# brown-palm/goal-force

Measured on AMD Instinct MI355X. Metric: frames_per_sec (81-frame video / (50-step denoise loop + VAE decode), Wan2.2-I2V-A14B 832x480x81f), higher is better.
Workload: dtype bf16

## Files before the change

goal_force_amd/csrc/gf_abi.hip:

```cpp
#include "gf_common.h"
#include <cstdarg>
#include <cstdio>
#include <cstdlib>
#include <cstring>

static thread_local char g_err[512] = "";

void gf_set_error(const char* fmt, ...) {
    va_list ap;
    va_start(ap, fmt);
    vsnprintf(g_err, sizeof(g_err), fmt, ap);
    va_end(ap);
}

extern "C" GF_API const char* gf_version(void) { return "goalforce-hip 0.1.0 gfx950"; }
extern "C" GF_API const char* gf_last_error(void) { return g_err; }
extern "C" GF_API int gf_abi_version(void) { return GF_ABI_VERSION; }

static GfOptions g_options;

const GfOptions& gf_options() { return g_options; }

namespace {
struct OptionSlot {
    const char* name;
    std::atomic<int> GfOptions::*field;
    int lo, hi, dflt;
};
const OptionSlot kSlots[] = {
    {"prefer_8wave", &GfOptions::prefer_8wave, 0, 1, 0}, {"a4_stagger", &GfOptions::a4_stagger, 0, 1 << 20, 2},
    {"a4_group_m", &GfOptions::a4_group_m, 0, 64, 0},    {"conv_nb", &GfOptions::conv_nb, 0, 2, 0},
    {"conv_gather", &GfOptions::conv_gather, 0, 1, 0},   {"vae_rms3", &GfOptions::vae_rms3, 0, 1, 1},
    {"conv_direct", &GfOptions::conv_direct, 0, 1, 1},
};
}

extern "C" GF_API int gf_set_option(const char* name, int value) {
    GF_CHECK_ARG(name, "gf_set_option: null name");
    for (const OptionSlot& s : kSlots)
        if (strcmp(name, s.name) == 0) {
            (g_options.*(s.field)).store(value < s.lo ? s.lo : (value > s.hi ? s.hi : value), std::memory_order_relaxed);
            return GF_OK;
        }
    gf_set_error("gf_set_option: unknown option '%s'", name);
    return GF_ERR_INVALID_ARG;
}

extern "C" GF_API int gf_get_option(const char* name, int* value) {
    GF_CHECK_ARG(name && value, "gf_get_option: null argument");
    for (const OptionSlot& s : kSlots)
        if (strcmp(name, s.name) == 0) {
            *value = (g_options.*(s.field)).load(std::memory_order_relaxed);
            return GF_OK;
        }
    gf_set_error("gf_get_option: unknown option '%s'", name);
    return GF_ERR_INVALID_ARG;
}

extern "C" GF_API void gf_reset_options(void) {
    for (const OptionSlot& s : kSlots) (g_options.*(s.field)).store(s.dflt, std::memory_order_relaxed);
}
```

goal_force_amd/csrc/gf_common.h:

```cpp
#pragma once
#include <hip/hip_runtime.h>
#include <stdint.h>
#include "goalforce.h"

typedef unsigned short u16;
typedef __attribute__((ext_vector_type(8))) __bf16 bf16x8;
typedef __attribute__((ext_vector_type(4))) __bf16 bf16x4;
typedef __attribute__((ext_vector_type(8))) unsigned short u16x8;
typedef __attribute__((ext_vector_type(4))) unsigned short u16x4;
typedef __attribute__((ext_vector_type(4))) short s16x4;
typedef __attribute__((ext_vector_type(4))) float f32x4;
typedef __attribute__((ext_vector_type(16))) float f32x16;
typedef __attribute__((ext_vector_type(4))) unsigned int u32x4;
typedef __attribute__((ext_vector_type(2))) unsigned int u32x2;

#define GF_LDS __attribute__((address_space(3)))
#define GF_GLOBAL __attribute__((address_space(1)))

__device__ __forceinline__ float bf2f(u16 u) { return __uint_as_float(((unsigned)u) << 16); }
__device__ __forceinline__ u16 f2bf(float f) { return __builtin_bit_cast(u16, (__bf16)f); }
__device__ __forceinline__ float rbf(float f) { return bf2f(f2bf(f)); }
__device__ __forceinline__ unsigned pack2bf(float lo, float hi) {
    typedef __attribute__((ext_vector_type(2))) float f2_t;
    typedef __attribute__((ext_vector_type(2))) __bf16 b2_t;
    return __builtin_bit_cast(unsigned, __builtin_convertvector(f2_t{lo, hi}, b2_t));
}

__device__ __forceinline__ float gelu_tanh_f(float x) {
    const float a = -2.0f * 0.7978845608028654f * 1.4426950408889634f, b = a * 0.044715f;
    const float t = __builtin_amdgcn_exp2f(x * __builtin_fmaf(b, x * x, a));
    return x * __builtin_amdgcn_rcpf(1.0f + t);
}
typedef __attribute__((ext_vector_type(2))) float gf_f32x2;
__device__ __forceinline__ void gelu_tanh_f4(gf_f32x2& x01, gf_f32x2& x23) {
    const float a = -2.0f * 0.7978845608028654f * 1.4426950408889634f, b = a * 0.044715f;
    const gf_f32x2 av = {a, a}, bv = {b, b}, one = {1.0f, 1.0f};
    const gf_f32x2 g01 = x01 * __builtin_elementwise_fma(bv, x01 * x01, av), g23 = x23 * __builtin_elementwise_fma(bv, x23 * x23, av);
    const float t0 = __builtin_amdgcn_exp2f(g01[0]), t1 = __builtin_amdgcn_exp2f(g01[1]);
    const float t2 = __builtin_amdgcn_exp2f(g23[0]), t3 = __builtin_amdgcn_exp2f(g23[1]);
    const gf_f32x2 d01 = one + gf_f32x2{t0, t1}, d23 = one + gf_f32x2{t2, t3};
    const float r0 = __builtin_amdgcn_rcpf(d01[0]), r1 = __builtin_amdgcn_rcpf(d01[1]);
    const float r2 = __builtin_amdgcn_rcpf(d23[0]), r3 = __builtin_amdgcn_rcpf(d23[1]);
    x01 = x01 * gf_f32x2{r0, r1};
    x23 = x23 * gf_f32x2{r2, r3};
}
__device__ __forceinline__ float silu_f(float x) { return x / (1.0f + __expf(-x)); }

__device__ __forceinline__ float wave_sum(float v) {
#pragma unroll
    for (int o = 32; o > 0; o >>= 1) v += __shfl_xor(v, o);
    return v;
}

template <int THREADS>
__device__ __forceinline__ float block_sum(float v, float* red) {
    v = wave_sum(v);
    const int w = threadIdx.x >> 6;
    __syncthreads();
    if ((threadIdx.x & 63) == 0) red[w] = v;
    __syncthreads();
    float t = 0.f;
#pragma unroll
    for (int i = 0; i < THREADS / 64; ++i) t += red[i];
    return t;
}

void gf_set_error(const char* fmt, ...);
#define GF_CHECK_ARG(cond, ...)                 \
    do {                                        \
        if (!(cond)) {                          \
            gf_set_error(__VA_ARGS__);          \
            return GF_ERR_INVALID_ARG;          \
        }                                       \
    } while (0)
#define GF_CHECK_LAUNCH(name)                                                        \
    do {                                                                             \
        hipError_t e_ = hipGetLastError();                                           \
        if (e_ != hipSuccess) {                                                      \
            gf_set_error("%s: launch failed: %s", name, hipGetErrorString(e_));      \
            return GF_ERR_LAUNCH;                                                    \
        }                                                                            \
    } while (0)
static inline bool gf_aligned16(const void* p) { return (((uintptr_t)p) & 15u) == 0; }

#include <atomic>
struct GfOptions {
    std::atomic<int> prefer_8wave{0};
    std::atomic<int> a4_stagger{2};
    std::atomic<int> a4_group_m{0};
    std::atomic<int> conv_nb{0};
    std::atomic<int> conv_gather{0};
    std::atomic<int> vae_rms3{1};
    std::atomic<int> conv_direct{1};
};
int gf_conv3d_direct_c96(const void* src_walk, const void* Wm, int64_t ldw, const void* bias, void* out, int64_t T_out, int64_t H,
                         int64_t W, int64_t N, int epilogue, const void* resid, const void* zero_page, void* stream);
int gf_conv2d_up_direct_c192(const void* src0, const void* Wm, int64_t ldw, const void* bias, void* out, int64_t T_out, int64_t Hs,
                             int64_t Ws, const void* zero_page, void* stream);
const GfOptions& gf_options();

#include <atomic>
#include <mutex>
struct GfDeviceOnce {
    std::atomic<uint64_t> done{0};
    std::mutex mu;
};
template <class F>
static inline hipError_t gf_once_per_device(GfDeviceOnce& st, F&& f) {
    int dev = 0;
    hipError_t e = hipGetDevice(&dev);
    if (e != hipSuccess) return e;
    if (dev < 0 || dev >= 64) return hipErrorInvalidDevice;
    const uint64_t bit = 1ull << dev;
    if (st.done.load(std::memory_order_acquire) & bit) return hipSuccess;
    std::lock_guard<std::mutex> lock(st.mu);
    if (st.done.load(std::memory_order_relaxed) & bit) return hipSuccess;
    e = f();
    if (e == hipSuccess) st.done.fetch_or(bit, std::memory_order_release);
    return e;
}
```

goal_force_amd/csrc/gf_gemm.hip:

```cpp
#include "gf_common.h"
#include <cstdlib>
#include <type_traits>


namespace {

constexpr int BM = 256, BN = 256, BK = 64;
constexpr int GEMM_THREADS = 512;
constexpr int TILE_BYTES = BM * BK * 2;
constexpr int STAGE_BYTES = 2 * TILE_BYTES;
constexpr int GEMM_LDS = 2 * STAGE_BYTES;
constexpr int GROUP_M = 8;

struct ConvGeom {
    const u16* src;
    const u16* cache;
    const u16* zero;
    int H, W, C, Ho, Wo, kt, ks, mode, t_stride, t_off, taps;
    int hist_front;
    int c64;
    long frame;
    float inv_c, inv_ks2;
};

// ... 547 lines not shown
#pragma unroll
        for (int j = 0; j < 2; ++j) {
            if (b && j >= J1) continue;
            const int ncol = (NB == 3 && b) ? 128 + wc * 16 + fq * 4 : b * 128 + wc * 32 + j * 16 + fq * 4;
            float bv[4] = {0.f, 0.f, 0.f, 0.f};
            if (p.bias && n0 + ncol < p.N) {
                const u16x4 b4 = *reinterpret_cast<const u16x4*>(p.bias + n0 + ncol);
#pragma unroll
                for (int r = 0; r < 4; ++r) bv[r] = bf2f(b4[r]);
            }
#pragma unroll
            for (int a = 0; a < 2; ++a)
#pragma unroll
                for (int i = 0; i < 4; ++i) {
                    const int row = a * 128 + wr * 64 + i * 16 + frow;
                    float rs = 1.0f;
                    if constexpr (FP8) rs = p.row_scale[min(m0 + row, p.M - 1)];
                    float y[4];
#pragma unroll
                    for (int r = 0; r < 4; ++r) {
                        y[r] = gf_epi_act<EPI>(acc[a][b][i][j][r] * rs + bv[r]);
                    }
                    u32x2 pk;
                    pk[0] = pack2bf(y[0], y[1]);
                    pk[1] = pack2bf(y[2], y[3]);
                    const int slot = (ncol >> 2) ^ ((row & 15) << 1);
                    *(GF_LDS u32x2*)(lds + row * 512 + slot * 8) = pk;
                }
        }
    __syncthreads();
    {
        const int cc = lane & 31;
        const int n = n0 + cc * 8;
        const bool n_ok = n < p.N && cc * 8 < BNT;
        u16x8 g8;
        if (EPI == GF_EPI_BIAS_GATE_RESID && n_ok) g8 = *reinterpret_cast<const u16x8*>(p.gate + n);
#pragma unroll
        for (int it = 0; it < 16; ++it) {
            const int row = wave * 32 + it * 2 + (lane >> 5);
            const int m = m0 + row;
            const u16x8 yv = *(GF_LDS u16x8*)(lds + row * 512 + ((cc ^ (row & 15)) << 4));
            if (m < p.M && n_ok) {
                u16x8 o = yv;
                if (EPI == GF_EPI_BIAS_GATE_RESID || EPI == GF_EPI_BIAS_RESID || EPI == GF_EPI_BIAS_MUL) {
                    const u16x8 r8 = rpre[HAS_R ? it : 0];
#pragma unroll
                    for (int e = 0; e < 8; ++e) {
                        float t = bf2f(yv[e]);
                        if (EPI == GF_EPI_BIAS_GATE_RESID) t = rbf(bf2f(g8[e]) * t);
                        o[e] = (EPI == GF_EPI_BIAS_MUL) ? f2bf(t * bf2f(r8[e]))
                                                        : f2bf(bf2f(r8[e]) + t);
                    }
                }
                *reinterpret_cast<u16x8*>(pC + (long)m * p.ldc + n) = o;
            }
        }
    }
}

#include "gf_gemm_a4_loop.inc"
#include "gf_gemm_a4f8_loop.inc"
constexpr int A4_THREADS = 256;

template <int I>
__device__ __forceinline__ float a4_acc() {
    float x;
    asm volatile("v_accvgpr_read_b32 %0, a[%1]" : "=v"(x) : "n"(I));
    return x;
}
template <int I, int N, class F>
__device__ __forceinline__ void a4_static_for(F&& f) {
    if constexpr (I < N) {
        f(std::integral_constant<int, I>{});
        a4_static_for<I + 1, N>(f);
    }
}

template <int EPI, bool FP8 = false>
__global__ __launch_bounds__(A4_THREADS, 1) void gemm_a4_kernel(const GemmArgs p) {
    constexpr unsigned ESZ = FP8 ? 1u : 2u;
    extern __shared__ __attribute__((aligned(16))) char smem[];
    GF_LDS char* lds = (GF_LDS char*)smem;
    const int tid = threadIdx.x;
    const int lane = tid & 63;
    const int wave = __builtin_amdgcn_readfirstlane(tid >> 6);
    const int wm = wave >> 1, wn = wave & 1;

    const int nwg = p.tiles_m * p.tiles_n;
    int v;
    {
        const int pid = blockIdx.x;
        const int xcd = pid & 7, local = pid >> 3;
        const int q = nwg >> 3, r = nwg & 7;
        v = (xcd < r ? xcd * (q + 1) : r * (q + 1) + (xcd - r) * q) + local;
    }
    const int gm = p.group_m;
    const int per_group = gm * p.tiles_n;
    const int group = v / per_group;
    const int first_m = group * gm;
    const int gsz = min(p.tiles_m - first_m, gm);
    const int in_group = v - group * per_group;
    const int m0 = (first_m + in_group % gsz) * BM, n0 = (in_group / gsz) * BN;

    const int srow = lane >> 3;
    unsigned voffA = (unsigned)srow * (unsigned)p.lda * ESZ + (unsigned)(((lane & 7) ^ srow) << 4);
    unsigned voffB = (unsigned)srow * (unsigned)p.ldw * ESZ + (unsigned)(((lane & 7) ^ srow) << 4);
    unsigned pfA = (unsigned)lane * (unsigned)p.lda * ESZ, pfB = (unsigned)lane * (unsigned)p.ldw * ESZ;
    const unsigned long baseA = (unsigned long)((const char*)p.A + (long)m0 * p.lda * ESZ);
    const unsigned long baseB = (unsigned long)((const char*)p.W + (long)n0 * p.ldw * ESZ);
    const unsigned aLo = (unsigned)baseA, aHi = (unsigned)(baseA >> 32) & 0xffffu;
    const unsigned bLo = (unsigned)baseB, bHi = (unsigned)(baseB >> 32) & 0xffffu;
    const unsigned nrA = (unsigned)(((long)(min(p.M - m0, BM) - 1) * p.lda + p.K) * ESZ);
    const int wvalid = min(p.wrows - n0, BN);
    const unsigned nrB = wvalid > 0 ? (unsigned)(((long)(wvalid - 1) * p.ldw + p.K) * ESZ) : 0u;
    const unsigned stA = 32u * (unsigned)p.lda * ESZ, stB = 32u * (unsigned)p.ldw * ESZ;
    const unsigned soA = (unsigned)wave * 8u * (unsigned)p.lda * ESZ, soB = (unsigned)wave * 8u * (unsigned)p.ldw * ESZ;
    const unsigned ldsW = (unsigned)(unsigned long)lds + (unsigned)wave * 1024u;
    const unsigned nk = (unsigned)(p.K * (int)ESZ / 128);
    const unsigned k0 = p.stagger ? (unsigned)((p.stagger * (p.stagger_rows ? m0 / BM : n0 / BN)) % (int)nk) : 0u;
    const unsigned kb = (unsigned)p.K * ESZ;

    const int frow = lane & 15, fq = lane >> 4, sw = frow & 7;
    const unsigned lbase = (unsigned)(unsigned long)lds;
    unsigned rdA0 = lbase + (unsigned)((wm * 128 + frow) * 128 + (((0 + fq) ^ sw) << 4));
    unsigned rdA1 = lbase + (unsigned)((wm * 128 + frow) * 128 + (((4 + fq) ^ sw) << 4));
    unsigned rdB0 = lbase + (unsigned)(TILE_BYTES + (wn * 128 + frow) * 128 + (((0 + fq) ^ sw) << 4));
    unsigned rdB1 = lbase + (unsigned)(TILE_BYTES + (wn * 128 + frow) * 128 + (((4 + fq) ^ sw) << 4));

    u16x4 bpre[8];
    u16x8 gpre = {0, 0, 0, 0, 0, 0, 0, 0};
    {
        const int fq_ = lane >> 4;
#pragma unroll
        for (int j = 0; j < 8; ++j) {
            const int n = n0 + wn * 128 + j * 16 + fq_ * 4;
            bpre[j] = (EPI != GF_EPI_VT32 && p.bias && n < p.N) ? *reinterpret_cast<const u16x4*>(p.bias + n) : u16x4{0, 0, 0, 0};
        }
        const int ng = n0 + wn * 128 + (lane & 15) * 8;
        if (EPI == GF_EPI_BIAS_GATE_RESID && ng < p.N) gpre = *reinterpret_cast<const u16x8*>(p.gate + ng);
        if (EPI == GF_EPI_VT32 && p.bias) {
#pragma unroll
            for (int i = 0; i < 8; ++i) {
                const int mrow = m0 + wm * 128 + i * 16 + (lane & 15);
                if (mrow < p.M) bpre[i][0] = p.bias[mrow];
            }
        }
    }
    float rsc[FP8 ? 8 : 1];
    if constexpr (FP8 && EPI != GF_EPI_VT32) {
#pragma unroll
        for (int i = 0; i < 8; ++i) rsc[i] = p.row_scale[min(m0 + wm * 128 + i * 16 + (lane & 15), p.M - 1)];
    }
    if constexpr (FP8) {
        GF_A4F8_LOOP_ASM(voffA, voffB, rdA0, rdA1, rdB0, rdB1, aLo, aHi, nrA, bLo, bHi, nrB, soA, stA, soB, stB, ldsW, nk, k0, kb);
    } else
    {
        GF_A4_LOOP_ASM(voffA, voffB, pfA, pfB, rdA0, rdA1, rdB0, rdB1, aLo, aHi, nrA, bLo, bHi, nrB, soA, stA, soB, stB, ldsW, nk, k0, kb);
    }

    GF_LDS char* ep = lds + wave * 32768;
    constexpr bool HAS_R = EPI == GF_EPI_BIAS_GATE_RESID || EPI == GF_EPI_BIAS_RESID || EPI == GF_EPI_BIAS_MUL;
    u16x8 rres[HAS_R ? 32 : 1];
    if constexpr (HAS_R) {
        const int nr = n0 + wn * 128 + (lane & 15) * 8;
#pragma unroll
        for (int it = 0; it < 32; ++it) {
            const int mr = m0 + wm * 128 + it * 4 + (lane >> 4);
            if (mr < p.M && nr < p.N) {
                rres[it] = __builtin_nontemporal_load(reinterpret_cast<const u16x8*>(p.R + (long)mr * p.ldr + nr));
            } else {
                rres[it] = u16x8{0, 0, 0, 0, 0, 0, 0, 0};
            }
        }
    }
    f32x4 csc[(FP8 && EPI == GF_EPI_VT32) ? 8 : 1];
    if constexpr (FP8 && EPI == GF_EPI_VT32) {
#pragma unroll
        for (int j = 0; j < 8; ++j) {
            const int n = n0 + wn * 128 + j * 16 + fq * 4;
#pragma unroll
            for (int r = 0; r < 4; ++r) csc[j][r] = (n + r < p.wrows) ? p.row_scale[n + r] : 0.f;
        }
    }
    a4_static_for<0, 8>([&](auto j_c) {
        constexpr int j = decltype(j_c)::value;
        const int n = n0 + wn * 128 + j * 16 + fq * 4;
        const float bv[4] = {bf2f(bpre[j][0]), bf2f(bpre[j][1]), bf2f(bpre[j][2]), bf2f(bpre[j][3])};
        a4_static_for<0, 8>([&](auto i_c) {
            constexpr int i = decltype(i_c)::value;
            constexpr int A0 = (i * 8 + j) * 4;
            float y[4] = {a4_acc<A0>(), a4_acc<A0 + 1>(), a4_acc<A0 + 2>(), a4_acc<A0 + 3>()};
            if constexpr (FP8 && EPI != GF_EPI_VT32) {
#pragma unroll
                for (int r = 0; r < 4; ++r) y[r] = y[r] * rsc[i] + bv[r];
            }
            if constexpr (EPI == GF_EPI_VT32) {
                const float bm = bf2f(bpre[i][0]);
                if constexpr (FP8) {
#pragma unroll
                    for (int r = 0; r < 4; ++r) y[r] = (n + r < p.wrows) ? y[r] * csc[j][r] + bm : 0.f;
                } else {
#pragma unroll
                    for (int r = 0; r < 4; ++r) y[r] = (n + r < p.wrows) ? y[r] + bm : 0.f;
                }
            } else if constexpr (EPI == GF_EPI_BIAS_GELU_TANH) {
                const unsigned l01 = FP8 ? pack2bf(y[0], y[1]) : pack2bf(y[0] + bv[0], y[1] + bv[1]);
                const unsigned l23 = FP8 ? pack2bf(y[2], y[3]) : pack2bf(y[2] + bv[2], y[3] + bv[3]);
                gf_f32x2 g01 = {__uint_as_float(l01 << 16), __uint_as_float(l01 & 0xffff0000u)};
                gf_f32x2 g23 = {__uint_as_float(l23 << 16), __uint_as_float(l23 & 0xffff0000u)};
                gelu_tanh_f4(g01, g23);
                y[0] = g01[0];
                y[1] = g01[1];
                y[2] = g23[0];
                y[3] = g23[1];
            } else {
#pragma unroll
                for (int r = 0; r < 4; ++r) {
                    y[r] = gf_epi_act<EPI>(FP8 ? y[r] : y[r] + bv[r]);
                }
            }
            u32x2 pk;
            pk[0] = pack2bf(y[0], y[1]);
            pk[1] = pack2bf(y[2], y[3]);
            const int row = i * 16 + frow;
            const int slot = (j * 4 + fq) ^ ((row & 15) << 1);
            *(GF_LDS u32x2*)(ep + row * 256 + slot * 8) = pk;
        });
    });
    asm volatile("s_waitcnt lgkmcnt(0)" ::: "memory");
    {
        const int cc = lane & 15;
        const int n = n0 + wn * 128 + cc * 8;
        const bool n_ok = n < p.N;
        const u16x8 g8 = gpre;
#pragma unroll
        for (int it = 0; it < 32; ++it) {
            const int row = it * 4 + (lane >> 4);
            const int m = m0 + wm * 128 + row;
            u16x8 yv;
            if constexpr (EPI == GF_EPI_VT32) {
                const int G = cc >> 2, g = cc & 3, sw = (row & 15) << 1;
                const u16x4 lo = *(GF_LDS u16x4*)(ep + row * 256 + (((8 * G + g) ^ sw) << 3));
                const u16x4 hi = *(GF_LDS u16x4*)(ep + row * 256 + (((8 * G + 4 + g) ^ sw) << 3));
                yv = u16x8{lo[0], lo[1], lo[2], lo[3], hi[0], hi[1], hi[2], hi[3]};
            } else {
                yv = *(GF_LDS u16x8*)(ep + row * 256 + ((cc ^ (row & 15)) << 4));
            }
            if (m < p.M && n_ok) {
                u16x8 o = yv;
                if constexpr (HAS_R) {
                    const u16x8 r8 = rres[it];
#pragma unroll
                    for (int e = 0; e < 8; ++e) {
                        float t = bf2f(yv[e]);
                        if (EPI == GF_EPI_BIAS_GATE_RESID) t = rbf(bf2f(g8[e]) * t);
                        o[e] = (EPI == GF_EPI_BIAS_MUL) ? f2bf(t * bf2f(r8[e]))
                                                        : f2bf(bf2f(r8[e]) + t);
                    }
                }
                __builtin_nontemporal_store(o, reinterpret_cast<u16x8*>(p.C + (long)m * p.ldc + n));
            }
        }
    }
}

template <int EPI, bool FP8 = false>
int launch_gemm_a4(const GemmArgs& a0, hipStream_t stream) {
    GemmArgs a = a0;
    {
        const int g = gf_options().a4_group_m.load(std::memory_order_relaxed);
        a.group_m = g > 0 ? g : (a.K * (FP8 ? 1 : 2) >= 16384 ? 4 : GROUP_M);
    }
    static GfDeviceOnce once;
    hipError_t e = gf_once_per_device(once, [] {
        return hipFuncSetAttribute(reinterpret_cast<const void*>(gemm_a4_kernel<EPI, FP8>),
                                   hipFuncAttributeMaxDynamicSharedMemorySize, GEMM_LDS);
    });
    if (e != hipSuccess) {
        gf_set_error("gf_gemm: hipFuncSetAttribute(%d B LDS) failed: %s", GEMM_LDS, hipGetErrorString(e));
        return GF_ERR_LAUNCH;
    }
    hipLaunchKernelGGL((gemm_a4_kernel<EPI, FP8>), dim3((unsigned)(a.tiles_m * a.tiles_n)), dim3(A4_THREADS), GEMM_LDS, stream, a);
    GF_CHECK_LAUNCH(FP8 ? "gf_gemm_fp8" : "gf_gemm_bf16");
    return GF_OK;
}

template <int EPI, bool FP8>
int launch_gemm(const GemmArgs& a, hipStream_t stream) {
    const bool use_a4 = gf_options().prefer_8wave.load(std::memory_order_relaxed) == 0;
    if constexpr (!FP8) {
        if (use_a4 && a.M >= 512 && a.K % 64 == 0 && 256L * a.lda * 2 + a.K * 2L < (1L << 31) &&
            256L * a.ldw * 2 + a.K * 2L < (1L << 31))
            return launch_gemm_a4<EPI>(a, stream);
    } else {
        if (use_a4 && a.M >= 512 && a.K % 128 == 0 && 256L * a.lda + a.K < (1L << 31) && 256L * a.ldw + a.K < (1L << 31))
            return launch_gemm_a4<EPI, true>(a, stream);
    }
    static GfDeviceOnce once;
    hipError_t e = gf_once_per_device(once, [] {
        const void* fn;
        if constexpr (FP8) fn = reinterpret_cast<const void*>(gemm_kernel<EPI, true>);
        else fn = reinterpret_cast<const void*>(gemm_ph_kernel<EPI, false>);
        return hipFuncSetAttribute(fn, hipFuncAttributeMaxDynamicSharedMemorySize, GEMM_LDS);
    });
    if (e != hipSuccess) {
        gf_set_error("gf_gemm: hipFuncSetAttribute(%d B LDS) failed: %s", GEMM_LDS, hipGetErrorString(e));
        return GF_ERR_LAUNCH;
    }
    if constexpr (FP8)
        hipLaunchKernelGGL((gemm_kernel<EPI, true>), dim3((unsigned)(a.tiles_m * a.tiles_n)), dim3(GEMM_THREADS), GEMM_LDS, stream, a);
    else
        hipLaunchKernelGGL((gemm_ph_kernel<EPI, false>), dim3((unsigned)(a.tiles_m * a.tiles_n)), dim3(GEMM_THREADS), GEMM_LDS,
                           stream, a);
    GF_CHECK_LAUNCH(FP8 ? "gf_gemm_fp8" : "gf_gemm_bf16");
    return GF_OK;
}

template <int EPI, int NB, int CONV>
int launch_conv(const GemmArgs& a, hipStream_t stream, int batch = 1) {
    static GfDeviceOnce once;
    hipError_t e = gf_once_per_device(once, [] {
        return hipFuncSetAttribute(reinterpret_cast<const void*>(gemm_ph_kernel<EPI, false, CONV, NB>),
                                   hipFuncAttributeMaxDynamicSharedMemorySize, GEMM_LDS);
    });
    if (e != hipSuccess) {
        gf_set_error("gf_conv3d: hipFuncSetAttribute(%d B LDS) failed: %s", GEMM_LDS, hipGetErrorString(e));
        return GF_ERR_LAUNCH;
    }
    hipLaunchKernelGGL((gemm_ph_kernel<EPI, false, CONV, NB>), dim3((unsigned)(a.tiles_m * a.tiles_n), (unsigned)batch), dim3(GEMM_THREADS),
                       GEMM_LDS, stream, a);
    GF_CHECK_LAUNCH("gf_conv3d_bf16");
    return GF_OK;
}

}
__device__ __attribute__((used, visibility("default"))) u16 gf_conv_zero_page[128] = {};
namespace {

const u16* conv_zero_page() {
    static GfDeviceOnce once;
    static const u16* page[64] = {};
    int dev = 0;
    if (hipGetDevice(&dev) != hipSuccess || dev < 0 || dev >= 64) return nullptr;
    hipError_t e = gf_once_per_device(once, [dev] {
        void* z = nullptr;
        hipError_t r = hipGetSymbolAddress(&z, HIP_SYMBOL(gf_conv_zero_page));
        if (r == hipSuccess) page[dev] = (const u16*)z;
        return r;
    });
    return e == hipSuccess ? page[dev] : nullptr;
}

}

static int gemm_dispatch(bool fp8, const void* A, int64_t lda, const void* W, int64_t ldw, const float* row_scale,
                         const void* bias, void* C, int64_t ldc, int64_t M, int64_t N, int64_t K, int epilogue,
                         const void* resid, int64_t ldr, const void* gate, void* stream) {
    const char* fn = fp8 ? "gf_gemm_fp8" : "gf_gemm_bf16";
    const int bke = fp8 ? 128 : 64, lal = fp8 ? 16 : 8;
    GF_CHECK_ARG(A && W && C, "%s: null A/W/C", fn);
    GF_CHECK_ARG(M >= 0 && N > 0 && K > 0, "%s: bad sizes M=%ld N=%ld K=%ld", fn, (long)M, (long)N, (long)K);
    GF_CHECK_ARG(K % bke == 0, "%s: K=%ld must be a multiple of %d", fn, (long)K, bke);
    GF_CHECK_ARG(N % 8 == 0, "%s: N=%ld must be a multiple of 8", fn, (long)N);
    GF_CHECK_ARG(lda % lal == 0 && ldw % lal == 0 && ldc % 8 == 0 && lda >= K && ldw >= K && ldc >= N,
                 "%s: leading dimensions must be multiples of %d (A/W) / 8 (C) and cover the row", fn, lal);
// ... 260 lines not shown
```

goal_force_amd/ops.py:

```python
from __future__ import annotations

import math

import torch

from . import _lib
from ._lib import (EPI_BIAS, EPI_BIAS_GATE_RESID, EPI_BIAS_GELU_TANH, EPI_BIAS_MUL, EPI_BIAS_RESID, EPI_BIAS_SILU,
                   GoalForceError)

__all__ = [
    "modulation", "layernorm_modulate", "rmsnorm_rope", "gate_residual", "gemm", "flash_attn", "flash_attn_sparse", "BlockMap", "patchify_im2col", "unpatchify",
    "cfg_euler_step", "act", "add", "sub", "rel_l1", "force_map",
    "EPI_BIAS", "EPI_BIAS_GELU_TANH", "EPI_BIAS_GATE_RESID", "EPI_BIAS_RESID", "EPI_BIAS_SILU", "EPI_BIAS_MUL",
]

_BF16 = torch.bfloat16
_FP8 = torch.float8_e4m3fn

PROFILE_ATTN = None
PROFILE_GEMM = None
PROFILE_CONV = None


def _stream(t: torch.Tensor):
# ... 137 lines not shown
def rmsnorm_rope(x, weight, cos=None, sin=None, head_dim=128, eps=1e-6):
    _req(x, "rmsnorm_rope.x")
    _req(weight, "rmsnorm_rope.weight")
    xv, rows, dim, xs = _rows2d(x, "rmsnorm_rope.x")
    if cos is not None:
        _req(cos, "rmsnorm_rope.cos", torch.float32)
        _req(sin, "rmsnorm_rope.sin", torch.float32)
        if cos.shape != (rows, head_dim // 2) or sin.shape != cos.shape or not cos.is_contiguous() \
                or not sin.is_contiguous():
            raise GoalForceError(f"rmsnorm_rope: cos/sin must be contiguous [{rows}, {head_dim // 2}]")
    _lib.check(_lib.load().gf_rmsnorm_rope(_ptr(xv), _ptr(weight), _ptr(cos), _ptr(sin), rows, dim, head_dim, xs,
                                           float(eps), _stream(x)), "gf_rmsnorm_rope")
    return x


def modulate(x, shift, scale):
    _req(x, "modulate.x")
    xv, rows, dim, xs = _rows2d(x, "modulate.x")
    _vec(shift, "modulate.shift", dim, required=True)
    _vec(scale, "modulate.scale", dim, required=True)
    out = torch.empty(x.shape, dtype=_BF16, device=x.device)
    ov, _, _, os_ = _rows2d(out, "modulate.out")
    _lib.check(_lib.load().gf_modulate(_ptr(xv), _ptr(ov), _ptr(scale), _ptr(shift), rows, dim, xs, os_, _stream(x)), "gf_modulate")
    return out


def gate_residual(x, gate, residual):
    _req(x, "gate_residual.x")
    _req(residual, "gate_residual.residual")
    xv, rows, dim, xs = _rows2d(x, "gate_residual.x")
    rv, rrows, rdim, rs = _rows2d(residual, "gate_residual.residual")
    if (rrows, rdim) != (rows, dim):
        raise GoalForceError(f"gate_residual: residual must match x [{rows}, {dim}]")
    _vec(gate, "gate_residual.gate", dim, required=True)
    out = torch.empty(x.shape, dtype=_BF16, device=x.device)
    ov, _, _, os_ = _rows2d(out, "gate_residual.out")
    _lib.check(_lib.load().gf_gate_residual(_ptr(xv), _ptr(gate), _ptr(rv), _ptr(ov), rows, dim, xs, rs, os_, _stream(x)),
               "gf_gate_residual")
    return out


def rope_apply(x, cos, sin, head_dim):
    _req(x, "rope_apply.x")
    xv, rows, dim, xs = _rows2d(x, "rope_apply.x")
    for n, t in (("cos", cos), ("sin", sin)):
        _req(t, f"rope_apply.{n}", torch.float32)
        if tuple(t.shape) != (rows, head_dim // 2) or not t.is_contiguous():
            raise GoalForceError(f"rope_apply.{n}: expected contiguous [{rows}, {head_dim // 2}] fp32")
    out = torch.empty(x.shape, dtype=_BF16, device=x.device)
    ov, _, _, os_ = _rows2d(out, "rope_apply.out")
    _lib.check(_lib.load().gf_rope_apply(_ptr(xv), _ptr(ov), _ptr(cos), _ptr(sin), rows, dim, head_dim, xs, os_, _stream(x)),
               "gf_rope_apply")
    return out


def _gemm(a, w, row_scale, bias, epilogue, resid, gate, out):
    av, M, K, lda, N, ldw = _linear_operands(a, w, row_scale)
    if out is None:
        out = torch.empty(a.shape[:-1] + (N,), dtype=_BF16, device=a.device)
    ov, Mo, No, ldc = _rows2d(out, "gemm[_fp8].out")
    if (Mo, No) != (M, N):
        raise GoalForceError(f"gemm[_fp8].out: expected [{M}, {N}], got [{Mo}, {No}]")
    ldr = 0
    if resid is not None:
        _req(resid, "gemm[_fp8].resid")
        resid, Mr, Nr, ldr = _rows2d(resid, "gemm[_fp8].resid")
        if (Mr, Nr) != (M, N):
            raise GoalForceError(f"gemm[_fp8].resid: expected [{M}, {N}], got [{Mr}, {Nr}]")
    _vec(gate, "gemm[_fp8].gate", N)
    _vec(bias, "gemm[_fp8].bias", N)
    lib = _lib.load()
    fn, scale = (lib.gf_gemm_bf16, ()) if row_scale is None else (lib.gf_gemm_fp8, (_ptr(row_scale),))
    with _timed(PROFILE_GEMM, M, N, K, int(epilogue)):
        _lib.check(fn(_ptr(av), lda, _ptr(w), ldw, *scale, _ptr(bias), _ptr(ov), ldc, M, N, K, int(epilogue), _ptr(resid), ldr,
                      _ptr(gate), _stream(a)), fn.__name__)
    return out


def gemm(a, w, bias=None, epilogue=EPI_BIAS, resid=None, gate=None, out=None):
    return _gemm(a, w, None, bias, epilogue, resid, gate, out)


VT_MIN_KV = 2048
_LIB_DEFAULTS = {"prefer_8wave": 0, "a4_stagger": 2, "a4_group_m": 0, "conv_nb": 0, "conv_gather": 0, "conv_direct": 1, "vae_rms3": 1}
_OPT = {"attn_k3": True, "vt_from_gemm": True, "conv_padded": True, "fold_pad_keys": True, "attn_q_prescale": True, "vae_attn_offset": True,
        "fold_cross_o": True}


def lib_option(name: str) -> int:
    import ctypes
    v = ctypes.c_int(0)
    _lib.check(_lib.load().gf_get_option(name.encode(), ctypes.byref(v)), f"gf_get_option({name})")
    return int(v.value)


class options:

    def __init__(self, **kv):
        for k in kv:
            if k not in _OPT and k not in _LIB_DEFAULTS:
                raise GoalForceError(f"ops.options: unknown option {k!r}")
        self.kv, self.old = kv, {}

    @staticmethod
    def _apply_one(k, v):
        if k in _OPT:
            _OPT[k] = bool(v)
        else:
            _lib.check(_lib.load().gf_set_option(k.encode(), int(v)), f"gf_set_option({k})")

    def __enter__(self):
        self.old = {}
        try:
            for k, v in self.kv.items():
                old = _OPT[k] if k in _OPT else lib_option(k)
                self._apply_one(k, v)
                self.old[k] = old
        except BaseException:
            self.__exit__(None, None, None)
            raise
        return self

    def __exit__(self, *exc):
        for k, v in reversed(list(self.old.items())):
            self._apply_one(k, v)
        self.old = {}
        return False


_VT_WS = {}


def _vt_workspace(numel, device):
    key = (device.index, torch.cuda.current_stream(device).cuda_stream)
    ws = _VT_WS.get(key)
    if ws is None or ws.numel() < numel:
        ws = _VT_WS[key] = torch.empty((numel,), dtype=_BF16, device=device)
    return ws


def _vt_shape(skv, num_heads, head_dim):
    return skv >= VT_MIN_KV and head_dim == 128 and num_heads * 128 * kv_pad(skv) < 2 ** 31


def vt32_ok(skv, num_heads, head_dim):
    return _vt_shape(skv, num_heads, head_dim) and _OPT["attn_k3"] and _OPT["vt_from_gemm"]


def _linear_vt32(x, w, x_scale, bias):
    xv, skv, K, ldx, N, ldw = _linear_operands(x, w, x_scale)
    _vec(bias, "linear_vt32[_fp8].bias", N)
    vt = _vt_workspace(N * kv_pad(skv), x.device)
    lib = _lib.load()
    fn, scale = (lib.gf_linear_vt32, ()) if x_scale is None else (lib.gf_linear_vt32_fp8, (_ptr(x_scale),))
    _lib.check(fn(_ptr(xv), ldx, *scale, _ptr(w), ldw, _ptr(bias), _ptr(vt), skv, kv_pad(skv), N, K, _stream(x)), fn.__name__)
    return vt


def linear_vt32(x, weight, bias):
    return _linear_vt32(x, weight, None, bias)


def linear_vt32_fp8(x8, x_scale, w8, bias):
    if x_scale is None:
        raise GoalForceError("linear_vt32_fp8.x_scale: required")
    return _linear_vt32(x8, w8, x_scale, bias)

# ... 814 lines not shown
```

Baseline: 0.6335.

## Make the a4 GEMM kernel persistent with a CU-sized grid looping over tiles

The 256x256 a4 GEMM kernel becomes persistent. It launches at most one workgroup per CU (rounded down to a multiple of 8 for the XCD mapping) and each workgroup loops over output tiles with a grid stride, with a barrier between tiles so epilogue LDS reuse is safe. The goal is to cut tail and launch-wave imbalance when the tile count is not a multiple of the CU count, and to amortize workgroup setup. In exchange each tile runs serially inside a workgroup, the XCD-aware tile remap is now applied to a strided tile index, and register pressure rises from the loop structure. A new option, on by default, controls it.

```diff
diff --git a/goal_force_amd/csrc/gf_abi.hip b/goal_force_amd/csrc/gf_abi.hip
--- a/goal_force_amd/csrc/gf_abi.hip
+++ b/goal_force_amd/csrc/gf_abi.hip
@@ -31,7 +31,7 @@
     {"prefer_8wave", &GfOptions::prefer_8wave, 0, 1, 0}, {"a4_stagger", &GfOptions::a4_stagger, 0, 1 << 20, 2},
     {"a4_group_m", &GfOptions::a4_group_m, 0, 64, 0},    {"conv_nb", &GfOptions::conv_nb, 0, 2, 0},
     {"conv_gather", &GfOptions::conv_gather, 0, 1, 0},   {"vae_rms3", &GfOptions::vae_rms3, 0, 1, 1},
-    {"conv_direct", &GfOptions::conv_direct, 0, 1, 1},
+    {"conv_direct", &GfOptions::conv_direct, 0, 1, 1},   {"a4_persistent", &GfOptions::a4_persistent, 0, 1, 1},
 };
 }
 
diff --git a/goal_force_amd/csrc/gf_common.h b/goal_force_amd/csrc/gf_common.h
--- a/goal_force_amd/csrc/gf_common.h
+++ b/goal_force_amd/csrc/gf_common.h
@@ -88,6 +88,7 @@
     std::atomic<int> prefer_8wave{0};
     std::atomic<int> a4_stagger{2};
     std::atomic<int> a4_group_m{0};
+    std::atomic<int> a4_persistent{1};
     std::atomic<int> conv_nb{0};
     std::atomic<int> conv_gather{0};
     std::atomic<int> vae_rms3{1};
diff --git a/goal_force_amd/csrc/gf_gemm.hip b/goal_force_amd/csrc/gf_gemm.hip
--- a/goal_force_amd/csrc/gf_gemm.hip
+++ b/goal_force_amd/csrc/gf_gemm.hip
@@ -653,171 +653,181 @@
     extern __shared__ __attribute__((aligned(16))) char smem[];
     GF_LDS char* lds = (GF_LDS char*)smem;
     const int tid = threadIdx.x;
-    const int lane = tid & 63;
     const int wave = __builtin_amdgcn_readfirstlane(tid >> 6);
     const int wm = wave >> 1, wn = wave & 1;
 
     const int nwg = p.tiles_m * p.tiles_n;
-    int v;
-    {
-        const int pid = blockIdx.x;
-        const int xcd = pid & 7, local = pid >> 3;
-        const int q = nwg >> 3, r = nwg & 7;
-        v = (xcd < r ? xcd * (q + 1) : r * (q + 1) + (xcd - r) * q) + local;
-    }
     const int gm = p.group_m;
     const int per_group = gm * p.tiles_n;
-    const int group = v / per_group;
-    const int first_m = group * gm;
-    const int gsz = min(p.tiles_m - first_m, gm);
-    const int in_group = v - group * per_group;
-    const int m0 = (first_m + in_group % gsz) * BM, n0 = (in_group / gsz) * BN;
-
-    const int srow = lane >> 3;
-    unsigned voffA = (unsigned)srow * (unsigned)p.lda * ESZ + (unsigned)(((lane & 7) ^ srow) << 4);
-    unsigned voffB = (unsigned)srow * (unsigned)p.ldw * ESZ + (unsigned)(((lane & 7) ^ srow) << 4);
-    unsigned pfA = (unsigned)lane * (unsigned)p.lda * ESZ, pfB = (unsigned)lane * (unsigned)p.ldw * ESZ;
-    const unsigned long baseA = (unsigned long)((const char*)p.A + (long)m0 * p.lda * ESZ);
-    const unsigned long baseB = (unsigned long)((const char*)p.W + (long)n0 * p.ldw * ESZ);
-    const unsigned aLo = (unsigned)baseA, aHi = (unsigned)(baseA >> 32) & 0xffffu;
-    const unsigned bLo = (unsigned)baseB, bHi = (unsigned)(baseB >> 32) & 0xffffu;
-    const unsigned nrA = (unsigned)(((long)(min(p.M - m0, BM) - 1) * p.lda + p.K) * ESZ);
-    const int wvalid = min(p.wrows - n0, BN);
-    const unsigned nrB = wvalid > 0 ? (unsigned)(((long)(wvalid - 1) * p.ldw + p.K) * ESZ) : 0u;
     const unsigned stA = 32u * (unsigned)p.lda * ESZ, stB = 32u * (unsigned)p.ldw * ESZ;
     const unsigned soA = (unsigned)wave * 8u * (unsigned)p.lda * ESZ, soB = (unsigned)wave * 8u * (unsigned)p.ldw * ESZ;
     const unsigned ldsW = (unsigned)(unsigned long)lds + (unsigned)wave * 1024u;
     const unsigned nk = (unsigned)(p.K * (int)ESZ / 128);
-    const unsigned k0 = p.stagger ? (unsigned)((p.stagger * (p.stagger_rows ? m0 / BM : n0 / BN)) % (int)nk) : 0u;
     const unsigned kb = (unsigned)p.K * ESZ;
-
-    const int frow = lane & 15, fq = lane >> 4, sw = frow & 7;
     const unsigned lbase = (unsigned)(unsigned long)lds;
-    unsigned rdA0 = lbase + (unsigned)((wm * 128 + frow) * 128 + (((0 + fq) ^ sw) << 4));
-    unsigned rdA1 = lbase + (unsigned)((wm * 128 + frow) * 128 + (((4 + fq) ^ sw) << 4));
-    unsigned rdB0 = lbase + (unsigned)(TILE_BYTES + (wn * 128 + frow) * 128 + (((0 + fq) ^ sw) << 4));
-    unsigned rdB1 = lbase + (unsigned)(TILE_BYTES + (wn * 128 + frow) * 128 + (((4 + fq) ^ sw) << 4));
-
-    u16x4 bpre[8];
-    u16x8 gpre = {0, 0, 0, 0, 0, 0, 0, 0};
-    {
-        const int fq_ = lane >> 4;
-#pragma unroll
-        for (int j = 0; j < 8; ++j) {
-            const int n = n0 + wn * 128 + j * 16 + fq_ * 4;
-            bpre[j] = (EPI != GF_EPI_VT32 && p.bias && n < p.N) ? *reinterpret_cast<const u16x4*>(p.bias + n) : u16x4{0, 0, 0, 0};
-        }
-        const int ng = n0 + wn * 128 + (lane & 15) * 8;
-        if (EPI == GF_EPI_BIAS_GATE_RESID && ng < p.N) gpre = *reinterpret_cast<const u16x8*>(p.gate + ng);
-        if (EPI == GF_EPI_VT32 && p.bias) {
+
+    for (int t = blockIdx.x; t < nwg; t += gridDim.x) {
+        int lane;
+        asm volatile("v_mbcnt_lo_u32_b32 %0, -1, 0\n\tv_mbcnt_hi_u32_b32 %0, -1, %0" : "=v"(lane));
+        const int srow = lane >> 3;
+        const int frow = lane & 15, fq = lane >> 4, sw = frow & 7;
+        int v;
+        {
+            const int pid = t;
+            const int xcd = pid & 7, local = pid >> 3;
+            const int q = nwg >> 3, r = nwg & 7;
+            v = (xcd < r ? xcd * (q + 1) : r * (q + 1) + (xcd - r) * q) + local;
+        }
+        const int group = v / per_group;
+        const int first_m = group * gm;
+        const int gsz = min(p.tiles_m - first_m, gm);
+        const int in_group = v - group * per_group;
+        const int m0 = (first_m + in_group % gsz) * BM, n0 = (in_group / gsz) * BN;
+
+        unsigned voffA = (unsigned)srow * (unsigned)p.lda * ESZ + (unsigned)(((lane & 7) ^ srow) << 4);
+        unsigned voffB = (unsigned)srow * (unsigned)p.ldw * ESZ + (unsigned)(((lane & 7) ^ srow) << 4);
+        unsigned pfA = (unsigned)lane * (unsigned)p.lda * ESZ, pfB = (unsigned)lane * (unsigned)p.ldw * ESZ;
+        const unsigned long baseA = (unsigned long)((const char*)p.A + (long)m0 * p.lda * ESZ);
+        const unsigned long baseB = (unsigned long)((const char*)p.W + (long)n0 * p.ldw * ESZ);
+        const unsigned aLo = (unsigned)baseA, aHi = (unsigned)(baseA >> 32) & 0xffffu;
+        const unsigned bLo = (unsigned)baseB, bHi = (unsigned)(baseB >> 32) & 0xffffu;
+        const unsigned nrA = (unsigned)(((long)(min(p.M - m0, BM) - 1) * p.lda + p.K) * ESZ);
+        const int wvalid = min(p.wrows - n0, BN);
+        const unsigned nrB = wvalid > 0 ? (unsigned)(((long)(wvalid - 1) * p.ldw + p.K) * ESZ) : 0u;
+        const unsigned k0 = p.stagger ? (unsigned)((p.stagger * (p.stagger_rows ? m0 / BM : n0 / BN)) % (int)nk) : 0u;
+
+        unsigned rdA0 = lbase + (unsigned)((wm * 128 + frow) * 128 + (((0 + fq) ^ sw) << 4));
+        unsigned rdA1 = lbase + (unsigned)((wm * 128 + frow) * 128 + (((4 + fq) ^ sw) << 4));
+        unsigned rdB0 = lbase + (unsigned)(TILE_BYTES + (wn * 128 + frow) * 128 + (((0 + fq) ^ sw) << 4));
+        unsigned rdB1 = lbase + (unsigned)(TILE_BYTES + (wn * 128 + frow) * 128 + (((4 + fq) ^ sw) << 4));
+
+        u16x4 bpre[8];
+        u16x8 gpre = {0, 0, 0, 0, 0, 0, 0, 0};
+        {
+            const int fq_ = lane >> 4;
+#pragma unroll
+            for (int j = 0; j < 8; ++j) {
+                const int n = n0 + wn * 128 + j * 16 + fq_ * 4;
+                bpre[j] = (EPI != GF_EPI_VT32 && p.bias && n < p.N) ? *reinterpret_cast<const u16x4*>(p.bias + n) : u16x4{0, 0, 0, 0};
+            }
+            const int ng = n0 + wn * 128 + (lane & 15) * 8;
+            if (EPI == GF_EPI_BIAS_GATE_RESID && ng < p.N) gpre = *reinterpret_cast<const u16x8*>(p.gate + ng);
+        }
+        unsigned rowb[EPI == GF_EPI_VT32 ? 8 : 1];
+        if constexpr (EPI == GF_EPI_VT32) {
 #pragma unroll
             for (int i = 0; i < 8; ++i) {
                 const int mrow = m0 + wm * 128 + i * 16 + (lane & 15);
-                if (mrow < p.M) bpre[i][0] = p.bias[mrow];
-            }
-        }
-    }
-    float rsc[FP8 ? 8 : 1];
-    if constexpr (FP8 && EPI != GF_EPI_VT32) {
-#pragma unroll
-        for (int i = 0; i < 8; ++i) rsc[i] = p.row_scale[min(m0 + wm * 128 + i * 16 + (lane & 15), p.M - 1)];
-    }
-    if constexpr (FP8) {
-        GF_A4F8_LOOP_ASM(voffA, voffB, rdA0, rdA1, rdB0, rdB1, aLo, aHi, nrA, bLo, bHi, nrB, soA, stA, soB, stB, ldsW, nk, k0, kb);
-    } else
-    {
-        GF_A4_LOOP_ASM(voffA, voffB, pfA, pfB, rdA0, rdA1, rdB0, rdB1, aLo, aHi, nrA, bLo, bHi, nrB, soA, stA, soB, stB, ldsW, nk, k0, kb);
-    }
-
-    GF_LDS char* ep = lds + wave * 32768;
-    constexpr bool HAS_R = EPI == GF_EPI_BIAS_GATE_RESID || EPI == GF_EPI_BIAS_RESID || EPI == GF_EPI_BIAS_MUL;
-    u16x8 rres[HAS_R ? 32 : 1];
-    if constexpr (HAS_R) {
-        const int nr = n0 + wn * 128 + (lane & 15) * 8;
-#pragma unroll
-        for (int it = 0; it < 32; ++it) {
-            const int mr = m0 + wm * 128 + it * 4 + (lane >> 4);
-            if (mr < p.M && nr < p.N) {
-                rres[it] = __builtin_nontemporal_load(reinterpret_cast<const u16x8*>(p.R + (long)mr * p.ldr + nr));
-            } else {
-                rres[it] = u16x8{0, 0, 0, 0, 0, 0, 0, 0};
-            }
-        }
-    }
-    f32x4 csc[(FP8 && EPI == GF_EPI_VT32) ? 8 : 1];
-    if constexpr (FP8 && EPI == GF_EPI_VT32) {
-#pragma unroll
-        for (int j = 0; j < 8; ++j) {
+                rowb[i] = (p.bias && mrow < p.M) ? p.bias[mrow] : 0u;
+            }
+        }
+        float rsc[FP8 ? 8 : 1];
+        if constexpr (FP8 && EPI != GF_EPI_VT32) {
+#pragma unroll
+            for (int i = 0; i < 8; ++i) rsc[i] = p.row_scale[min(m0 + wm * 128 + i * 16 + (lane & 15), p.M - 1)];
+        }
+        if constexpr (FP8) {
+            GF_A4F8_LOOP_ASM(voffA, voffB, rdA0, rdA1, rdB0, rdB1, aLo, aHi, nrA, bLo, bHi, nrB, soA, stA, soB, stB, ldsW, nk, k0, kb);
+        } else
+        {
+            GF_A4_LOOP_ASM(voffA, voffB, pfA, pfB, rdA0, rdA1, rdB0, rdB1, aLo, aHi, nrA, bLo, bHi, nrB, soA, stA, soB, stB, ldsW, nk, k0, kb);
+        }
+        if constexpr (EPI == GF_EPI_VT32) {
+#pragma unroll
+            for (int i = 0; i < 8; ++i) asm volatile("" : "+v"(rowb[i]));
+        } else {
+#pragma unroll
+            for (int j = 0; j < 8; ++j) asm volatile("" : "+v"(bpre[j]));
+        }
+
+        GF_LDS char* ep = lds + wave * 32768;
+        constexpr bool HAS_R = EPI == GF_EPI_BIAS_GATE_RESID || EPI == GF_EPI_BIAS_RESID || EPI == GF_EPI_BIAS_MUL;
+        u16x8 rres[HAS_R ? 32 : 1];
+        if constexpr (HAS_R) {
+            const int nr = n0 + wn * 128 + (lane & 15) * 8;
+#pragma unroll
+            for (int it = 0; it < 32; ++it) {
+                const int mr = m0 + wm * 128 + it * 4 + (lane >> 4);
+                if (mr < p.M && nr < p.N) {
+                    rres[it] = __builtin_nontemporal_load(reinterpret_cast<const u16x8*>(p.R + (long)mr * p.ldr + nr));
+                } else {
+                    rres[it] = u16x8{0, 0, 0, 0, 0, 0, 0, 0};
+                }
+            }
+        }
+        f32x4 csc[(FP8 && EPI == GF_EPI_VT32) ? 8 : 1];
+        if constexpr (FP8 && EPI == GF_EPI_VT32) {
+#pragma unroll
+            for (int j = 0; j < 8; ++j) {
+                const int n = n0 + wn * 128 + j * 16 + fq * 4;
+#pragma unroll
+                for (int r = 0; r < 4; ++r) csc[j][r] = (n + r < p.wrows) ? p.row_scale[n + r] : 0.f;
+            }
+        }
+        a4_static_for<0, 8>([&](auto j_c) {
+            constexpr int j = decltype(j_c)::value;
             const int n = n0 + wn * 128 + j * 16 + fq * 4;
-#pragma unroll
-            for (int r = 0; r < 4; ++r) csc[j][r] = (n + r < p.wrows) ? p.row_scale[n + r] : 0.f;
-        }
-    }
-    a4_static_for<0, 8>([&](auto j_c) {
-        constexpr int j = decltype(j_c)::value;
-        const int n = n0 + wn * 128 + j * 16 + fq * 4;
-        const float bv[4] = {bf2f(bpre[j][0]), bf2f(bpre[j][1]), bf2f(bpre[j][2]), bf2f(bpre[j][3])};
-        a4_static_for<0, 8>([&](auto i_c) {
-            constexpr int i = decltype(i_c)::value;
-            constexpr int A0 = (i * 8 + j) * 4;
-            float y[4] = {a4_acc<A0>(), a4_acc<A0 + 1>(), a4_acc<A0 + 2>(), a4_acc<A0 + 3>()};
-            if constexpr (FP8 && EPI != GF_EPI_VT32) {
-#pragma unroll
-                for (int r = 0; r < 4; ++r) y[r] = y[r] * rsc[i] + bv[r];
-            }
-            if constexpr (EPI == GF_EPI_VT32) {
-                const float bm = bf2f(bpre[i][0]);
-                if constexpr (FP8) {
-#pragma unroll
-                    for (int r = 0; r < 4; ++r) y[r] = (n + r < p.wrows) ? y[r] * csc[j][r] + bm : 0.f;
+            const float bv[4] = {bf2f(bpre[j][0]), bf2f(bpre[j][1]), bf2f(bpre[j][2]), bf2f(bpre[j][3])};
+            a4_static_for<0, 8>([&](auto i_c) {
+                constexpr int i = decltype(i_c)::value;
+                constexpr int A0 = (i * 8 + j) * 4;
+                float y[4] = {a4_acc<A0>(), a4_acc<A0 + 1>(), a4_acc<A0 + 2>(), a4_acc<A0 + 3>()};
+                if constexpr (FP8 && EPI != GF_EPI_VT32) {
+#pragma unroll
+                    for (int r = 0; r < 4; ++r) y[r] = y[r] * rsc[i] + bv[r];
+                }
+                if constexpr (EPI == GF_EPI_VT32) {
+                    const float bm = bf2f((u16)rowb[i]);
+                    if constexpr (FP8) {
+#pragma unroll
+                        for (int r = 0; r < 4; ++r) y[r] = (n + r < p.wrows) ? y[r] * csc[j][r] + bm : 0.f;
+                    } else {
+#pragma unroll
+                        for (int r = 0; r < 4; ++r) y[r] = (n + r < p.wrows) ? y[r] + bm : 0.f;
+                    }
+                } else if constexpr (EPI == GF_EPI_BIAS_GELU_TANH) {
+                    const unsigned l01 = FP8 ? pack2bf(y[0], y[1]) : pack2bf(y[0] + bv[0], y[1] + bv[1]);
+                    const unsigned l23 = FP8 ? pack2bf(y[2], y[3]) : pack2bf(y[2] + bv[2], y[3] + bv[3]);
+                    gf_f32x2 g01 = {__uint_as_float(l01 << 16), __uint_as_float(l01 & 0xffff0000u)};
+                    gf_f32x2 g23 = {__uint_as_float(l23 << 16), __uint_as_float(l23 & 0xffff0000u)};
+                    gelu_tanh_f4(g01, g23);
+                    y[0] = g01[0];
+                    y[1] = g01[1];
+                    y[2] = g23[0];
+                    y[3] = g23[1];
                 } else {
 #pragma unroll
-                    for (int r = 0; r < 4; ++r) y[r] = (n + r < p.wrows) ? y[r] + bm : 0.f;
-                }
-            } else if constexpr (EPI == GF_EPI_BIAS_GELU_TANH) {
-                const unsigned l01 = FP8 ? pack2bf(y[0], y[1]) : pack2bf(y[0] + bv[0], y[1] + bv[1]);
-                const unsigned l23 = FP8 ? pack2bf(y[2], y[3]) : pack2bf(y[2] + bv[2], y[3] + bv[3]);
-                gf_f32x2 g01 = {__uint_as_float(l01 << 16), __uint_as_float(l01 & 0xffff0000u)};
-                gf_f32x2 g23 = {__uint_as_float(l23 << 16), __uint_as_float(l23 & 0xffff0000u)};
-                gelu_tanh_f4(g01, g23);
-                y[0] = g01[0];
-                y[1] = g01[1];
-                y[2] = g23[0];
-                y[3] = g23[1];
-            } else {
-#pragma unroll
-                for (int r = 0; r < 4; ++r) {
-                    y[r] = gf_epi_act<EPI>(FP8 ? y[r] : y[r] + bv[r]);
-                }
-            }
-            u32x2 pk;
-            pk[0] = pack2bf(y[0], y[1]);
-            pk[1] = pack2bf(y[2], y[3]);
-            const int row = i * 16 + frow;
-            const int slot = (j * 4 + fq) ^ ((row & 15) << 1);
-            *(GF_LDS u32x2*)(ep + row * 256 + slot * 8) = pk;
+                    for (int r = 0; r < 4; ++r) {
+                        y[r] = gf_epi_act<EPI>(FP8 ? y[r] : y[r] + bv[r]);
+                    }
+                }
+                u32x2 pk;
+                pk[0] = pack2bf(y[0], y[1]);
+                pk[1] = pack2bf(y[2], y[3]);
+                const int row = i * 16 + frow;
+                const int slot = (j * 4 + fq) ^ ((row & 15) << 1);
+                *(GF_LDS u32x2*)(ep + row * 256 + slot * 8) = pk;
+            });
         });
-    });
-    asm volatile("s_waitcnt lgkmcnt(0)" ::: "memory");
-    {
-        const int cc = lane & 15;
-        const int n = n0 + wn * 128 + cc * 8;
-        const bool n_ok = n < p.N;
-        const u16x8 g8 = gpre;
-#pragma unroll
-        for (int it = 0; it < 32; ++it) {
-            const int row = it * 4 + (lane >> 4);
-            const int m = m0 + wm * 128 + row;
-            u16x8 yv;
-            if constexpr (EPI == GF_EPI_VT32) {
-                const int G = cc >> 2, g = cc & 3, sw = (row & 15) << 1;
-                const u16x4 lo = *(GF_LDS u16x4*)(ep + row * 256 + (((8 * G + g) ^ sw) << 3));
-                const u16x4 hi = *(GF_LDS u16x4*)(ep + row * 256 + (((8 * G + 4 + g) ^ sw) << 3));
-                yv = u16x8{lo[0], lo[1], lo[2], lo[3], hi[0], hi[1], hi[2], hi[3]};
-            } else {
-                yv = *(GF_LDS u16x8*)(ep + row * 256 + ((cc ^ (row & 15)) << 4));
-            }
-            if (m < p.M && n_ok) {
+        asm volatile("s_waitcnt lgkmcnt(0)" ::: "memory");
+        {
+            const int cc = lane & 15;
+            const int n = n0 + wn * 128 + cc * 8;
+            const bool n_ok = n < p.N;
+            const u16x8 g8 = gpre;
+#pragma unroll
+            for (int it = 0; it < 32; ++it) {
+                const int row = it * 4 + (lane >> 4);
+                const int m = m0 + wm * 128 + row;
+                u16x8 yv;
+                if constexpr (EPI == GF_EPI_VT32) {
+                    const int G = cc >> 2, g = cc & 3, sw = (row & 15) << 1;
+                    const u16x4 lo = *(GF_LDS u16x4*)(ep + row * 256 + (((8 * G + g) ^ sw) << 3));
+                    const u16x4 hi = *(GF_LDS u16x4*)(ep + row * 256 + (((8 * G + 4 + g) ^ sw) << 3));
+                    yv = u16x8{lo[0], lo[1], lo[2], lo[3], hi[0], hi[1], hi[2], hi[3]};
+                } else {
+                    yv = *(GF_LDS u16x8*)(ep + row * 256 + ((cc ^ (row & 15)) << 4));
+                }
                 u16x8 o = yv;
                 if constexpr (HAS_R) {
                     const u16x8 r8 = rres[it];
@@ -828,11 +838,22 @@
                         o[e] = (EPI == GF_EPI_BIAS_MUL) ? f2bf(t * bf2f(r8[e]))
                                                         : f2bf(bf2f(r8[e]) + t);
                     }
-                }
-                __builtin_nontemporal_store(o, reinterpret_cast<u16x8*>(p.C + (long)m * p.ldc + n));
-            }
-        }
-    }
+                    asm volatile("" : "+v"(o));
+                }
+                if (m < p.M && n_ok) __builtin_nontemporal_store(o, reinterpret_cast<u16x8*>(p.C + (long)m * p.ldc + n));
+            }
+        }
+        asm volatile("s_waitcnt lgkmcnt(0)\n\ts_barrier" ::: "memory");
+    }
+}
+
+static int a4_cu_count() {
+    static GfDeviceOnce once;
+    static int cus[64] = {};
+    int dev = 0;
+    if (hipGetDevice(&dev) != hipSuccess || dev < 0 || dev >= 64) return 0;
+    hipError_t e = gf_once_per_device(once, [dev] { return hipDeviceGetAttribute(&cus[dev], hipDeviceAttributeMultiprocessorCount, dev); });
+    return e == hipSuccess ? cus[dev] : 0;
 }
 
 template <int EPI, bool FP8 = false>
@@ -851,7 +872,17 @@
         gf_set_error("gf_gemm: hipFuncSetAttribute(%d B LDS) failed: %s", GEMM_LDS, hipGetErrorString(e));
         return GF_ERR_LAUNCH;
     }
-    hipLaunchKernelGGL((gemm_a4_kernel<EPI, FP8>), dim3((unsigned)(a.tiles_m * a.tiles_n)), dim3(A4_THREADS), GEMM_LDS, stream, a);
+    const int tiles = a.tiles_m * a.tiles_n;
+    int grid = tiles;
+    if (gf_options().a4_persistent.load(std::memory_order_relaxed)) {
+        const int cus = a4_cu_count();
+        if (cus <= 0) {
+            gf_set_error("gf_gemm: hipDeviceGetAttribute(multiProcessorCount) failed");
+            return GF_ERR_LAUNCH;
+        }
+        if (tiles > cus) grid = cus >= 8 ? cus & ~7 : cus;
+    }
+    hipLaunchKernelGGL((gemm_a4_kernel<EPI, FP8>), dim3((unsigned)grid), dim3(A4_THREADS), GEMM_LDS, stream, a);
     GF_CHECK_LAUNCH(FP8 ? "gf_gemm_fp8" : "gf_gemm_bf16");
     return GF_OK;
 }
diff --git a/goal_force_amd/ops.py b/goal_force_amd/ops.py
--- a/goal_force_amd/ops.py
+++ b/goal_force_amd/ops.py
@@ -243,7 +243,7 @@
 
 
 VT_MIN_KV = 2048
-_LIB_DEFAULTS = {"prefer_8wave": 0, "a4_stagger": 2, "a4_group_m": 0, "conv_nb": 0, "conv_gather": 0, "conv_direct": 1, "vae_rms3": 1}
+_LIB_DEFAULTS = {"prefer_8wave": 0, "a4_stagger": 2, "a4_group_m": 0, "a4_persistent": 1, "conv_nb": 0, "conv_gather": 0, "conv_direct": 1, "vae_rms3": 1}
 _OPT = {"attn_k3": True, "vt_from_gemm": True, "conv_padded": True, "fold_pad_keys": True, "attn_q_prescale": True, "vae_attn_offset": True,
         "fold_cross_o": True}
 
```

Result: no change. 0.6334 (median of 2 runs) (-0.0%).
